# GinZhu/RDST

Measured on AMD Instinct MI355X. Metric: SR patches/sec fwd+bwd, RDST-E1 x4 64->256, higher is better.
Workload: dtype bf16; 1 GPU; RDST-E1 x4 (RDST_E1_OASIS_example_SRx4.ini), 1x64x64 LR patches -> 256x256, step = fwd + L1 + bwd + flat-bucket grad all-reduce + Adam; global_batch=32, per_gpu_batch=32, parallelism=dp1, hip_graph=True, grad_bucket_bytes=17859844

## Files before the change

### rdst_amd/csrc/mlp_mfma.hip

```cpp
#include "linear.h"
#include "mfma.h"
#include "reduce_batch.h"
#include "wattn_hd.h"
#include <stdlib.h>

#ifdef MLP_ABL
#define MLP_DBG(p) (MLP_ABL)
#else
#define MLP_DBG(p) RDST_DBGV((p).dbg)
#endif

namespace {
using namespace wahd;
using MM = Mma<bf16>;

struct MlpArgs {
  const bf16* X; int64_t ldx; const float* stats; const float* lnw; const float* lnb;
  const float* W1; const float* b1; const float* W2; const float* b2;
  const bf16* dY; int64_t lddy; bf16* dX; int64_t lddx;
  float* slab; int64_t slab_stride;
  int64_t M; int C; int hid; int64_t ntiles; int tiles_per_wg;
  unsigned long long* stamps;
  int dbg;
};

template <int NCT> struct MlpCfg {
  static constexpr int NJ = 2 * NCT, NT = 64 * NJ, CP = 32 * NCT, JP = 32 * NJ;
  static constexpr int KC = CP / 16, KJ = JP / 16, PK = CP / 8;
  static constexpr int LDW = NCT == 4 ? 336 : CP * 2 + 16, LDX = LDW, LDH = 64;
  static constexpr int OFF_W1 = 0, OFF_XH = OFF_W1 + JP * LDW, OFF_DY = OFF_XH + 32 * LDX, OFF_DH = OFF_DY + 32 * LDX,
                       OFF_B1 = OFF_DH + JP * LDH, OFF_SM = OFF_B1 + JP * 4, OFF_RED = OFF_SM + 32 * 4,
                       OFF_TAB = OFF_RED + NCT * 32 * 8, OFF_W2L = OFF_TAB + RDST_GELU_TAB_BYTES;
  static constexpr int W2L = NCT == 4 ? 3 : 0, SMEM = OFF_W2L + W2L * NJ * 1024;
};

__device__ __forceinline__ void gelu_pair(f32x2 x, f32x2& cdf, f32x2& ex) {
  const f32x2 z = x * 0.70710678118654752440f;
  f32x2 az;
  az.x = __builtin_fabsf(z.x); az.y = __builtin_fabsf(z.y);
  const f32x2 den = __builtin_elementwise_fma(az, (f32x2)(0.3275911f), (f32x2)(1.0f));
  f32x2 t;
  t.x = __builtin_amdgcn_rcpf(den.x); t.y = __builtin_amdgcn_rcpf(den.y);
  f32x2 pl = __builtin_elementwise_fma(t, (f32x2)(0.5f * 1.061405429f), (f32x2)(0.5f * -1.453152027f));
  pl = __builtin_elementwise_fma(pl, t, (f32x2)(0.5f * 1.421413741f));
  pl = __builtin_elementwise_fma(pl, t, (f32x2)(0.5f * -0.284496736f));
  pl = __builtin_elementwise_fma(pl, t, (f32x2)(0.5f * 0.254829592f));
  pl = pl * t;
  const f32x2 a2 = (z * -1.4426950408889634f) * z;
  ex.x = __builtin_amdgcn_exp2f(a2.x); ex.y = __builtin_amdgcn_exp2f(a2.y);
  const f32x2 qn = pl * ex, qp = (f32x2)(1.0f) - qn;
  cdf.x = x.x >= 0.f ? qp.x : qn.x;
  cdf.y = x.y >= 0.f ? qp.y : qn.y;
}

template <int NCT, bool SPLIT>
__global__ void __launch_bounds__(128 * NCT, 2) mlp_bwd_kernel(const MlpArgs p) {
  using CF = MlpCfg<NCT>;
  extern __shared__ __attribute__((aligned(16))) char smem[];
  constexpr int NT = CF::NT, JP = CF::JP, LDW = CF::LDW, LDX = CF::LDX, PK = CF::PK, NJ = CF::NJ;
  const int tid = threadIdx.x, lane = tid & 63, wave = __builtin_amdgcn_readfirstlane(tid >> 6), r = lane & 31, hh = lane >> 5;
  const int C = p.C, hid = p.hid;
  const int j = 32 * wave + r;
  float* b1s = reinterpret_cast<float*>(smem + CF::OFF_B1);
  float* sm = reinterpret_cast<float*>(smem + CF::OFF_SM);
  float* red = reinterpret_cast<float*>(smem + CF::OFF_RED);
  const lds_cp gtab = (lds_cp)(smem + CF::OFF_TAB);
  gelu_tab_fill(smem + CF::OFF_TAB, tid, NT);
  int nst = 0;
  auto stamp = [&]() {
    if (RDST_DBGV(p.stamps) && tid == 0 && nst < 14) p.stamps[(size_t)blockIdx.x * 16 + nst++] = __builtin_readcyclecounter();
  };
  stamp();

  Pack16 w2b[CF::KC - CF::W2L];
  const lds_cp w2l = (lds_cp)(smem + CF::OFF_W2L + (wave * 64 + lane) * 16);
  {
    float f[CF::KC][8];
#pragma unroll
    for (int t = 0; t < CF::KC; ++t)
#pragma unroll
      for (int e = 0; e < 8; ++e) {
        const int c = 16 * t + 8 * hh + e;
        f[t][e] = p.W2[(int64_t)(c < C ? c : C - 1) * hid + (j < hid ? j : hid - 1)];
      }
#pragma unroll
    for (int t = 0; t < CF::KC; ++t) {
#pragma unroll
      for (int e = 0; e < 8; ++e) f[t][e] = (16 * t + 8 * hh + e < C && j < hid) ? f[t][e] : 0.f;
      if (t < CF::KC - CF::W2L) w2b[t < CF::KC - CF::W2L ? t : 0] = MM::pack(f[t]);
      else {
        const Pack16 pk = MM::pack(f[t]);
        u32x4_t v; v.x = pk.w[0]; v.y = pk.w[1]; v.z = pk.w[2]; v.w = pk.w[3];
        *reinterpret_cast<LDS_AS u32x4_t*>(w2l + (t - (CF::KC - CF::W2L)) * NJ * 1024) = v;
      }
    }
  }
  stamp();
  lds_zero16(smem + CF::OFF_W1, CF::OFF_DH - CF::OFF_W1, tid, NT);
  const int pk = tid % PK, jr = tid / PK, c0 = 8 * pk;
  {
    float gq[8], bq[8];
#pragma unroll
    for (int e = 0; e < 8; ++e) {
      const int c = c0 + e < C ? c0 + e : C - 1;
      gq[e] = p.lnw[c];
      bq[e] = p.lnb[c];
    }
#pragma unroll
    for (int e = 0; e < 8; ++e) {
      gq[e] = c0 + e < C ? gq[e] : 0.f;
      bq[e] = c0 + e < C ? bq[e] : 0.f;
    }
    const int cl = c0 < C - 8 ? c0 : C - 8, sh = c0 - cl;
    float w[NJ][8];
#pragma unroll
    for (int ps = 0; ps < NJ; ++ps) {
      const int jj = jr + 32 * ps;
      const float* src = p.W1 + (int64_t)(jj < hid ? jj : hid - 1) * C + cl;
      const u32x4_a4 a = *reinterpret_cast<const u32x4_a4*>(src), b = *reinterpret_cast<const u32x4_a4*>(src + 4);
      w[ps][0] = __uint_as_float(a.x); w[ps][1] = __uint_as_float(a.y); w[ps][2] = __uint_as_float(a.z); w[ps][3] = __uint_as_float(a.w);
      w[ps][4] = __uint_as_float(b.x); w[ps][5] = __uint_as_float(b.y); w[ps][6] = __uint_as_float(b.z); w[ps][7] = __uint_as_float(b.w);
    }
    if (sh != 0) {
#pragma unroll
      for (int ps = 0; ps < NJ; ++ps) {
        float t4[8], t2[8];
#pragma unroll
        for (int e = 0; e < 8; ++e) t4[e] = (sh & 4) ? (e + 4 < 8 ? w[ps][e + 4 < 8 ? e + 4 : 7] : 0.f) : w[ps][e];
#pragma unroll
        for (int e = 0; e < 8; ++e) t2[e] = (sh & 2) ? (e + 2 < 8 ? t4[e + 2 < 8 ? e + 2 : 7] : 0.f) : t4[e];
#pragma unroll
        for (int e = 0; e < 8; ++e) w[ps][e] = sh >= 8 ? 0.f : t2[e];
      }
    }
    __syncthreads();
    stamp();
    float* part = reinterpret_cast<float*>(smem + CF::OFF_DH);
#pragma unroll
    for (int ps = 0; ps < NJ; ++ps) {
      const int jj = jr + 32 * ps;
      if (jj < hid) {
        float f[8], dot = 0.f;
#pragma unroll
        for (int e = 0; e < 8; ++e) {
          f[e] = w[ps][e] * gq[e];
          dot = fmaf(w[ps][e], bq[e], dot);
        }
        *reinterpret_cast<Pack16*>(smem + CF::OFF_W1 + jj * LDW + c0 * 2) = MM::pack(f);
        part[jj * PK + pk] = dot;
      }
    }
    if (tid < 32) *reinterpret_cast<uint16_t*>(smem + CF::OFF_XH + tid * LDX + C * 2) = 0x3f80;
  }
  __syncthreads();
  stamp();
  {
    const float* part = reinterpret_cast<const float*>(smem + CF::OFF_DH);
    for (int jj = tid; jj < JP; jj += NT) {
      float v = 0.f;
      if (jj < hid) {
        v = p.b1 ? p.b1[jj] : 0.f;
#pragma unroll
        for (int k = 0; k < PK; ++k) v += part[jj * PK + k];
      }
      b1s[jj] = v;
    }
  }
  __syncthreads();

  stamp();
  constexpr int NU = SPLIT ? 2 : 1;
  const bool loader = SPLIT ? wave >= NCT : true;
  const int rowbytes = C * 2;
  int lrow[NU], loff[NU];
  bool lact[NU], lal[NU], lfirst[NU];
  const char* xp[NU];
  const char* yp[NU];
  const float* sp[NU];
#pragma unroll
  for (int u = 0; u < NU; ++u) {
    const int idx = SPLIT ? (tid - 64 * NCT) + 64 * NCT * u : tid;
    lrow[u] = (idx / PK) & 31;
    const int chk = idx - (idx / PK) * PK;
    lact[u] = loader && chk * 16 < rowbytes;
    int o = chk * 16;
    if (o + 16 > rowbytes) o = rowbytes - 16;
    if (!lact[u]) o = 0;
    loff[u] = o;
    lal[u] = (o & 15) == 0;
    lfirst[u] = lact[u] && chk == 0;
  }
  u32x4_a4 rx[NU], rdy[NU];
  float2 rst[NU];
  auto seek = [&](int64_t tile) {
#pragma unroll
    for (int u = 0; u < NU; ++u) {
      int64_t row = tile * 32 + lrow[u];
      row = row < p.M ? row : p.M - 1;
      xp[u] = reinterpret_cast<const char*>(p.X + row * p.ldx) + loff[u];
      yp[u] = reinterpret_cast<const char*>(p.dY + row * p.lddy) + loff[u];
      sp[u] = p.stats + 2 * row;
    }
  };
  auto fetch = [&]() {
#pragma unroll
    for (int u = 0; u < NU; ++u) {
      rx[u] = *reinterpret_cast<const u32x4_a4*>(xp[u]);
      rdy[u] = *reinterpret_cast<const u32x4_a4*>(yp[u]);
      rst[u] = *reinterpret_cast<const float2*>(sp[u]);
    }
  };
  const int64_t xstep = 32 * p.ldx * 2, ystep = 32 * p.lddy * 2;
  auto advance = [&]() {
#pragma unroll
    for (int u = 0; u < NU; ++u) {
      xp[u] += xstep;
      yp[u] += ystep;
      sp[u] += 64;
    }
  };
  auto put16 = [&](char* dst, const Pack16& v, bool aligned) {
    if (aligned) *reinterpret_cast<Pack16*>(dst) = v;
    else {
      uint32_t* d = reinterpret_cast<uint32_t*>(dst);
      d[0] = v.w[0]; d[1] = v.w[1]; d[2] = v.w[2]; d[3] = v.w[3];
    }
  };
  auto stash = [&](int64_t tile) {
#pragma unroll
    for (int u = 0; u < NU; ++u) {
      const bool valid = tile * 32 + lrow[u] < p.M;
      if (lact[u]) {
        float f[8];
        unpack8(rx[u], f);
#pragma unroll
        for (int e = 0; e < 8; ++e) f[e] = valid ? (f[e] - rst[u].x) * rst[u].y : 0.f;
        put16(smem + CF::OFF_XH + lrow[u] * LDX + loff[u], MM::pack(f), lal[u]);
        Pack16 d;
        d.w[0] = valid ? rdy[u].x : 0u; d.w[1] = valid ? rdy[u].y : 0u; d.w[2] = valid ? rdy[u].z : 0u; d.w[3] = valid ? rdy[u].w : 0u;
        put16(smem + CF::OFF_DY + lrow[u] * LDX + loff[u], d, lal[u]);
      }
    }
#pragma unroll
    for (int u = 0; u < NU; ++u)
      if (lfirst[u]) sm[lrow[u]] = rst[u].y;
  };

  const int q = (lane & 15) >> 2, pp = lane & 3, gq1 = (lane >> 4) & 1;
  const int sg = (r & 16) + 4 * (r & 3) + ((r >> 2) & 1) + 2 * ((r >> 3) & 1);
  const lds_cp xrow = (lds_cp)(smem + CF::OFF_XH + sg * LDX + hh * 16);
  const lds_cp yrow = (lds_cp)(smem + CF::OFF_DY + sg * LDX + hh * 16);
  const lds_cp wrow = (lds_cp)(smem + CF::OFF_W1 + j * LDW + hh * 16);
  const int dhpos = 32 * wave + (r & 16) + 4 * (r & 3) + ((r >> 2) & 3);
  const uint32_t dho = (uint32_t)dhpos * CF::LDH + 8u * ((dhpos >> 1) & 7);
  const lds_cp dhb = (lds_cp)(smem + CF::OFF_DH);
  const lds_cp xtr = (lds_cp)(smem + CF::OFF_XH + (4 * q + hh) * LDX + (16 * gq1 + 4 * pp) * 2);
  const lds_cp ytr = (lds_cp)(smem + CF::OFF_DY + (4 * q + hh) * LDX + (16 * gq1 + 4 * pp) * 2);
  const lds_cp wtr = (lds_cp)(smem + CF::OFF_W1 + (4 * q + hh) * LDW + (16 * gq1 + 4 * pp) * 2 + wave * 64);
  const lds_cp dtr0 = dhb + (4 * hh + q) * CF::LDH + 8 * ((4 * gq1 + pp) ^ ((2 * hh + (q >> 1)) & 7));
  const lds_cp dtr1 = dhb + (4 * hh + 8 + q) * CF::LDH + 8 * ((4 * gq1 + pp) ^ ((2 * hh + 4 + (q >> 1)) & 7));
  static_assert(CF::LDH == 64 && CF::OFF_DH % 64 == 0, "dHp image: 64-byte rows, XOR swizzle of the 8-byte pieces");

  f32x16 G1[NCT], W2g[NCT];
#pragma unroll
  for (int ct = 0; ct < NCT; ++ct)
#pragma unroll
    for (int v = 0; v < 16; ++v) { G1[ct][v] = 0.f; W2g[ct][v] = 0.f; }

  const int64_t t0 = (int64_t)blockIdx.x * p.tiles_per_wg;
  const int64_t t1 = t0 + p.tiles_per_wg < p.ntiles ? t0 + p.tiles_per_wg : p.ntiles;
  const float invC = 1.0f / (float)C;
  const int64_t full_tiles = p.M / 32;
  if (loader && t0 < t1) {
    seek(t0);
    fetch();
  }
  for (int64_t tile = t0; tile < t1; ++tile) {
    if (loader) {
      stash(tile);
      if (tile + 1 < t1) {
        if (tile + 1 < full_tiles) advance();
        else seek(tile + 1);
      }
      fetch();
    }
    __syncthreads();
    stamp();
    Pack16 hA[2], dA[2];
    {
      f32x16 ah, ad;
      const float bj = b1s[j];
#pragma unroll
      for (int v = 0; v < 16; ++v) { ah[v] = bj; ad[v] = 0.f; }
      if (!(MLP_DBG(p) & 2))
#pragma unroll
      for (int t = 0; t < CF::KC; ++t) {
        const Pack16 xa = lds_pack(xrow + 32 * t), wb = lds_pack(wrow + 32 * t), ya = lds_pack(yrow + 32 * t);
        MM::mma(ah, xa, wb);
        if (t < CF::KC - CF::W2L) MM::mma(ad, ya, w2b[t < CF::KC - CF::W2L ? t : 0]);
        else MM::mma(ad, ya, lds_pack(w2l + (t - (CF::KC - CF::W2L)) * NJ * 1024));
      }
      const bool ones = j == hid;
#pragma unroll
      for (int s = 0; s < 2; ++s) {
        constexpr int LB = NCT == 4 ? 4 : 8;
#pragma unroll
        for (int b = 0; b < 8; b += LB) {
          float fr[LB];
          u32x2_t en[LB];
#pragma unroll
          for (int k = 0; k < LB; ++k) {
            uint32_t off;
            fr[k] = gelu_tab_index(ah[8 * s + b + k], off);
            if (MLP_DBG(p) & 1) { en[k].x = off; en[k].y = off + 1; }
            else en[k] = *reinterpret_cast<const LDS_AS u32x2_t*>(gtab + off);
          }
          __builtin_amdgcn_sched_barrier(0);
#pragma unroll
          for (int k = 0; k < LB; k += 2) {
            const int v = 8 * s + b + k;
            const float h0 = ah[v] * gelu_tab_lerp(fr[k], en[k].x), h1 = ah[v + 1] * gelu_tab_lerp(fr[k + 1], en[k + 1].x);
            const float d0 = ad[v] * gelu_tab_lerp(fr[k], en[k].y), d1 = ad[v + 1] * gelu_tab_lerp(fr[k + 1], en[k + 1].y);
            const uint32_t hp = pack_bf16x2(h0, h1);
            hA[s].w[(b + k) / 2] = ones ? 0x3f803f80u : hp;
            dA[s].w[(b + k) / 2] = pack_bf16x2(d0, d1);
          }
        }
        u32x2_t lo, hi;
        lo.x = dA[s].w[0]; lo.y = dA[s].w[1]; hi.x = dA[s].w[2]; hi.y = dA[s].w[3];
        *reinterpret_cast<LDS_AS u32x2_t*>(dhb + (dho ^ (uint32_t)(8 * (4 * s + hh)))) = lo;
        *reinterpret_cast<LDS_AS u32x2_t*>(dhb + (dho ^ (uint32_t)(8 * (4 * s + 2 + hh)))) = hi;
      }
    }
    __syncthreads();
    stamp();
    if (!(MLP_DBG(p) & 4))
#pragma unroll
    for (int ct = 0; ct < NCT; ++ct)
#pragma unroll
      for (int s = 0; s < 2; ++s) {
        const Pack16 xb = lds_tr_pack(xtr + 16 * s * LDX + ct * 64, xtr + (16 * s + 2) * LDX + ct * 64);
        const Pack16 yb = lds_tr_pack(ytr + 16 * s * LDX + ct * 64, ytr + (16 * s + 2) * LDX + ct * 64);
        MM::mma(G1[ct], dA[s], xb);
        MM::mma(W2g[ct], hA[s], yb);
      }
    f32x16 dx;
    float rstd = 0.f;
    if (wave < NCT) {
      f32x16 dx2;
#pragma unroll
      for (int v = 0; v < 16; ++v) { dx[v] = 0.f; dx2[v] = 0.f; }
      if (!(MLP_DBG(p) & 8))
#pragma unroll
      for (int kk = 0; kk < CF::KJ; kk += 2) {
        const Pack16 wa = lds_tr_pack(wtr + 16 * kk * LDW, wtr + (16 * kk + 2) * LDW);
        const Pack16 db = lds_tr_pack(dtr0 + 16 * kk * CF::LDH, dtr1 + 16 * kk * CF::LDH);
        const Pack16 wa2 = lds_tr_pack(wtr + 16 * (kk + 1) * LDW, wtr + (16 * (kk + 1) + 2) * LDW);
        const Pack16 db2 = lds_tr_pack(dtr0 + 16 * (kk + 1) * CF::LDH, dtr1 + 16 * (kk + 1) * CF::LDH);
        MM::mma(dx, wa, db);
        MM::mma(dx2, wa2, db2);
      }
#pragma unroll
      for (int v = 0; v < 16; ++v) dx[v] += dx2[v];
      rstd = sm[sg];
      float s1 = 0.f, s2 = 0.f;
#pragma unroll
      for (int g4 = 0; g4 < 4; ++g4) {
        const u32x2_t xv = *reinterpret_cast<const LDS_AS u32x2_t*>((lds_cp)(smem + CF::OFF_XH + sg * LDX) + (32 * wave + 8 * g4 + 4 * hh) * 2);
        const float xh[4] = {bf16lo(xv.x), bf16hi(xv.x), bf16lo(xv.y), bf16hi(xv.y)};
#pragma unroll
        for (int e = 0; e < 4; ++e) {
          s1 += dx[4 * g4 + e];
          s2 = fmaf(dx[4 * g4 + e], xh[e], s2);
        }
      }
      s1 = half_swap_sum(s1);
      s2 = half_swap_sum(s2);
      if (hh == 0) *reinterpret_cast<float2*>(red + (wave * 32 + r) * 2) = make_float2(s1, s2);
    }
    __syncthreads();
    stamp();
    if (wave < NCT) {
      float s1 = 0.f, s2 = 0.f;
#pragma unroll
      for (int w = 0; w < NCT; ++w) {
        const float2 v = *reinterpret_cast<const float2*>(red + (w * 32 + r) * 2);
        s1 += v.x; s2 += v.y;
      }
      s1 *= invC; s2 *= invC;
      float o[16];
#pragma unroll
      for (int g4 = 0; g4 < 4; ++g4) {
        const int cb = (32 * wave + 8 * g4 + 4 * hh) * 2;
        const u32x2_t xv = *reinterpret_cast<const LDS_AS u32x2_t*>((lds_cp)(smem + CF::OFF_XH + sg * LDX) + cb);
        const u32x2_t yv = *reinterpret_cast<const LDS_AS u32x2_t*>((lds_cp)(smem + CF::OFF_DY + sg * LDX) + cb);
        const float xh[4] = {bf16lo(xv.x), bf16hi(xv.x), bf16lo(xv.y), bf16hi(xv.y)};
        const float dy[4] = {bf16lo(yv.x), bf16hi(yv.x), bf16lo(yv.y), bf16hi(yv.y)};
#pragma unroll
        for (int e = 0; e < 4; ++e) o[4 * g4 + e] = fmaf(rstd, dx[4 * g4 + e] - s1 - xh[e] * s2, dy[e]);
      }
      const int64_t row = tile * 32 + sg;
      if (row < p.M) {
        bf16* drow = p.dX + row * p.lddx;
#pragma unroll
        for (int gp = 0; gp < 2; ++gp) {
          float c8[8];
#pragma unroll
          for (int e = 0; e < 4; ++e) {
            const auto sw = __builtin_amdgcn_permlane32_swap(__float_as_uint(o[8 * gp + e]), __float_as_uint(o[8 * gp + 4 + e]), false, false);
            c8[e] = __uint_as_float(sw[0]);
            c8[4 + e] = __uint_as_float(sw[1]);
          }
          const int cb = 32 * wave + 8 * (2 * gp + hh);
          if (cb + 8 <= C) {
            u32x4_a4 u;
            u.x = pack_bf16x2(c8[0], c8[1]); u.y = pack_bf16x2(c8[2], c8[3]);
            u.z = pack_bf16x2(c8[4], c8[5]); u.w = pack_bf16x2(c8[6], c8[7]);
            *reinterpret_cast<u32x4_a4*>(drow + cb) = u;
          } else {
#pragma unroll
            for (int e = 0; e < 8; ++e)
              if (cb + e < C) drow[cb + e] = __float2bfloat16(c8[e]);
          }
        }
      }
    }
    __syncthreads();
    stamp();
  }
  if (RDST_DBGV(p.stamps) && tid == 0) p.stamps[(size_t)blockIdx.x * 16 + 14] = __builtin_readcyclecounter();
  uint2* my = reinterpret_cast<uint2*>(p.slab) + (int64_t)blockIdx.x * p.slab_stride;
  uint2* my2 = my + (int64_t)((hid + 3) / 4) * (C + 1);
#pragma unroll
  for (int ct = 0; ct < NCT; ++ct) {
    const int c = 32 * ct + r;
#pragma unroll
    for (int g4 = 0; g4 < 4; ++g4) {
      const int j0 = 32 * wave + 8 * g4 + 4 * hh;
      if (j0 < hid && c <= C)
        my[(int64_t)(j0 >> 2) * (C + 1) + c] = make_uint2(pack_bf16x2(G1[ct][4 * g4], G1[ct][4 * g4 + 1]), pack_bf16x2(G1[ct][4 * g4 + 2], G1[ct][4 * g4 + 3]));
      if (j0 <= hid && c < C)
        my2[(int64_t)(j0 >> 2) * C + c] = make_uint2(pack_bf16x2(W2g[ct][4 * g4], W2g[ct][4 * g4 + 1]), pack_bf16x2(W2g[ct][4 * g4 + 2], W2g[ct][4 * g4 + 3]));
    }
  }
  if (RDST_DBGV(p.stamps) && tid == 0) p.stamps[(size_t)blockIdx.x * 16 + 15] = __builtin_readcyclecounter();
}

template <int NCT> struct MlpFwdCfg {
  static constexpr int NJ = 2 * NCT, NT = 64 * NJ, CP = 32 * NCT, JP = 32 * NJ;
  static constexpr int KC = CP / 16, KJ = JP / 16, PK = CP / 8;
  static constexpr int LDW = CP * 2 + 16, LDX = CP * 2 + 16, LD2 = JP * 2 + 16;
  static constexpr int off_w2(int hid) { return hid * LDW; }
  static constexpr int off_x(int hid, int C) { return off_w2(hid) + C * LD2; }
  static constexpr int off_h(int hid, int C) { return off_x(hid, C) + 32 * LDX; }
  static constexpr int off_pst(int hid, int C) { return off_h(hid, C) + 32 * LD2; }
  static constexpr int off_s(int hid, int C) { return off_pst(hid, C) + 32 * 16 * 8; }
  static constexpr int smem(int hid, int C) { return off_s(hid, C) + 2 * JP * 4 + CP * 4; }
};

struct MlpFwdArgs {
  const bf16* X; int64_t ldx; const float* lnw; const float* lnb;
  const float* W1; const float* b1; const float* W2; const float* b2;
  bf16* Y; int64_t ldy; float* stats;
  int64_t M; int C; int hid; int64_t ntiles; int tiles_per_wg;
  unsigned long long* stamps;
};

template <int NCT>
__global__ void __launch_bounds__(128 * NCT, 2) mlp_fwd_kernel(const MlpFwdArgs p) {
  using CF = MlpFwdCfg<NCT>;
  extern __shared__ __attribute__((aligned(16))) char smem[];
  constexpr int NT = CF::NT, JP = CF::JP, CP = CF::CP, LDW = CF::LDW, LDX = CF::LDX, LD2 = CF::LD2, PK = CF::PK, NJ = CF::NJ;
  const int tid = threadIdx.x, lane = tid & 63, wave = __builtin_amdgcn_readfirstlane(tid >> 6), r = lane & 31, hh = lane >> 5;
  const int C = p.C, hid = p.hid;
  const int OFF_W2 = CF::off_w2(hid), OFF_X = CF::off_x(hid, C), OFF_H = CF::off_h(hid, C), OFF_PST = CF::off_pst(hid, C),
            OFF_S = CF::off_s(hid, C);
  float* Ss = reinterpret_cast<float*>(smem + OFF_S);
  float* b1s = Ss + JP;
  float* b2s = b1s + JP;
  float2* pst = reinterpret_cast<float2*>(smem + OFF_PST);
  int nst = 0;
  auto stamp = [&]() {
    if (RDST_DBGV(p.stamps) && tid == 0 && nst < 16) p.stamps[(size_t)blockIdx.x * 16 + nst++] = __builtin_readcyclecounter();
  };
  stamp();

  lds_zero16(smem, OFF_H, tid, NT);
  const int pk = tid % PK, jr = tid / PK, c0 = 8 * pk;
  {
    float gq[8], bq[8];
#pragma unroll
    for (int e = 0; e < 8; ++e) {
      const int c = c0 + e < C ? c0 + e : C - 1;
      gq[e] = p.lnw[c];
      bq[e] = p.lnb[c];
    }
// ... 204 lines not shown
        const int kc = 2 * k + hh;
        const bool last = kc == nchunk - 1;
        const float d = q2[k].x * (last ? inv_nlast : 0.125f) - mean;
        m2 += kc < nchunk ? fmaf((last ? (float)nlast : 8.0f) * d, d, q2[k].y) : 0.f;
      }
      m2 = half_swap_sum(m2);
#pragma unroll
      for (int v = 0; v < 16; ++v) ah[v] += ah2[v];
      const float rstd = 1.0f / sqrtf(m2 * invC + 1e-5f);
      const int64_t row = tile * 32 + r;
      if (wave == 0 && hh == 0 && row < p.M) *reinterpret_cast<float2*>(p.stats + 2 * row) = make_float2(mean, rstd);
      const float nm = -mean * rstd;
#pragma unroll
      for (int g4 = 0; g4 < 4; ++g4) {
        const float sq[4] = {Sr[4 * g4], Sr[4 * g4 + 1], Sr[4 * g4 + 2], Sr[4 * g4 + 3]};
        const float bq[4] = {B1r[4 * g4], B1r[4 * g4 + 1], B1r[4 * g4 + 2], B1r[4 * g4 + 3]};
        float hv[4];
#pragma unroll
        for (int e2 = 0; e2 < 2; ++e2) {
          f32x2 x, cdf, ex;
          x.x = fmaf(ah[4 * g4 + 2 * e2], rstd, fmaf(nm, sq[2 * e2], bq[2 * e2]));
          x.y = fmaf(ah[4 * g4 + 2 * e2 + 1], rstd, fmaf(nm, sq[2 * e2 + 1], bq[2 * e2 + 1]));
          gelu_pair(x, cdf, ex);
          hv[2 * e2] = x.x * cdf.x;
          hv[2 * e2 + 1] = x.y * cdf.y;
        }
        u32x2_t w2;
        w2.x = pack_bf16x2(hv[0], hv[1]); w2.y = pack_bf16x2(hv[2], hv[3]);
        *reinterpret_cast<LDS_AS u32x2_t*>(hwr + 16 * g4) = w2;
      }
    }
    __syncthreads();
    stamp();
    if (wave < NCT) {
      f32x16 y0, y1;
#pragma unroll
      for (int v = 0; v < 16; ++v) { y0[v] = B2r[v]; y1[v] = 0.f; }
#pragma unroll
      for (int kk = 0; kk < CF::KJ; kk += 2) {
        const Pack16 wa = lds_pack(w2row + 32 * kk), hb = lds_pack(hrd + 32 * kk);
        const Pack16 wa2 = lds_pack(w2row + 32 * (kk + 1)), hb2 = lds_pack(hrd + 32 * (kk + 1));
        MM::mma(y0, wa, hb);
        MM::mma(y1, wa2, hb2);
      }
      float o[16];
#pragma unroll
      for (int g4 = 0; g4 < 4; ++g4) {
        const u32x2_t xv = *reinterpret_cast<const LDS_AS u32x2_t*>((lds_cp)(smem + OFF_X + r * LDX) + (j0 + 8 * g4 + 4 * hh) * 2);
        const float xr[4] = {bf16lo(xv.x), bf16hi(xv.x), bf16lo(xv.y), bf16hi(xv.y)};
#pragma unroll
        for (int e = 0; e < 4; ++e) o[4 * g4 + e] = y0[4 * g4 + e] + y1[4 * g4 + e] + xr[e];
      }
      const int64_t row = tile * 32 + r;
      if (row < p.M) {
        bf16* yrow = p.Y + row * p.ldy;
#pragma unroll
        for (int gp = 0; gp < 2; ++gp) {
          float c8[8];
#pragma unroll
          for (int e = 0; e < 4; ++e) {
            const auto sw = __builtin_amdgcn_permlane32_swap(__float_as_uint(o[8 * gp + e]), __float_as_uint(o[8 * gp + 4 + e]), false, false);
            c8[e] = __uint_as_float(sw[0]);
            c8[4 + e] = __uint_as_float(sw[1]);
          }
          const int cb = j0 + 8 * (2 * gp + hh);
          if (cb + 8 <= C) {
            u32x4_a4 u;
            u.x = pack_bf16x2(c8[0], c8[1]); u.y = pack_bf16x2(c8[2], c8[3]);
            u.z = pack_bf16x2(c8[4], c8[5]); u.w = pack_bf16x2(c8[6], c8[7]);
            *reinterpret_cast<u32x4_a4*>(yrow + cb) = u;
          } else {
#pragma unroll
            for (int e = 0; e < 8; ++e)
              if (cb + e < C) yrow[cb + e] = __float2bfloat16(c8[e]);
          }
        }
      }
    }
    __syncthreads();
    stamp();
  }
}

int mlp_nct(int C, int hid) {
  const int nct = (C + 1 + 31) / 32;
  if (nct < 2 || nct > 4) return 0;
  if (hid + 1 > 64 * nct || hid < 32) return 0;
  if ((C & 1) || C * 2 < 16) return 0;
  const int fs = nct == 2 ? MlpFwdCfg<2>::smem(hid, C) : nct == 3 ? MlpFwdCfg<3>::smem(hid, C) : MlpFwdCfg<4>::smem(hid, C);
  if (fs > 160 * 1024) return 0;
  return nct;
}

bool mlp_fused(int C, int hid) {
  static int off = -1;
  if (off < 0) {
    const char* e = rdst_dbg_getenv("RDST_MLP_V1");
    off = (e && e[0] == '1') ? 1 : 0;
  }
  return !off && mlp_nct(C, hid) != 0;
}

}

extern "C" int rdst_mlp_fused_supported(int C, int hid, int dtype) {
  if (rdst_dtype(dtype, "rdst_mlp_fused_supported")) return 0;
  return dtype == RDST_BF16 && mlp_fused(C, hid);
}

namespace {
struct MlpBwdWs {
  WsSlab slab;
  float* G;
  size_t bytes;
};
MlpBwdWs mlp_bwd_layout(void* base, int C, int hid) {
  WsCarver c(base);
  MlpBwdWs w{};
  w.slab = ws_take_slab(c, 2 * kCUs, (int64_t)hid * (C + 1) + (int64_t)(hid + 1) * C);
  w.G = c.take<float>((size_t)hid * (C + 1) + kWsSlackFloats);
  w.bytes = c.bytes();
  return w;
}
}

extern "C" size_t rdst_mlp_bwd_workspace(int64_t M, int C, int hid) {
  (void)M;
  if (C <= 0 || hid <= 0) return 0;
  return mlp_bwd_layout(nullptr, C, hid).bytes;
}

extern "C" int rdst_mlp_bwd(const void* X, int64_t ld_x, const float* ln_w, const float* ln_b, const float* stats,
                            const float* W1, const float* b1, const float* W2, const void* dY, int64_t ld_dy, void* dX,
                            int64_t ld_dx, float* dW1, float* db1, float* dW2, float* db2, float* dln_w, float* dln_b,
                            void* workspace, size_t workspace_bytes, int64_t M, int C, int hid, int dtype, void* stream) {
  if (int rc = rdst_dtype(dtype, "rdst_mlp_bwd")) return rc;
  if (!X || !ln_w || !ln_b || !stats || !W1 || !W2 || !dY || !dX || !dW1 || !db1 || !dW2 || !db2 || !dln_w || !dln_b || !workspace)
    return rdst_fail(RDST_EINVAL, "rdst_mlp_bwd: null pointer");
  if (M < 0 || C <= 0 || hid <= 0 || ld_x < C || ld_dy < C || ld_dx < C) return rdst_fail(RDST_EINVAL, "rdst_mlp_bwd: bad dimensions");
  if (dtype != RDST_BF16 || !mlp_fused(C, hid)) return RDST_ENOTSUP;
  if (((uintptr_t)X & 3) || ((uintptr_t)dY & 3) || ((uintptr_t)dX & 3) || (ld_x & 1) || (ld_dy & 1) || (ld_dx & 1)) return RDST_ENOTSUP;
  if (workspace_bytes < rdst_mlp_bwd_workspace(M, C, hid)) return rdst_fail(RDST_EINVAL, "rdst_mlp_bwd: workspace too small");
  if (M == 0) return 0;
  hipStream_t st = (hipStream_t)stream;
  const int nct = mlp_nct(C, hid);
  MlpArgs p{};
  p.X = (const bf16*)X; p.ldx = ld_x; p.stats = stats; p.lnw = ln_w; p.lnb = ln_b; p.W1 = W1; p.b1 = b1; p.W2 = W2;
  p.dY = (const bf16*)dY; p.lddy = ld_dy; p.dX = (bf16*)dX; p.lddx = ld_dx;
  p.M = M; p.C = C; p.hid = hid;
  p.ntiles = (M + 31) / 32;
  int64_t cap = nct == 2 ? 2 * kCUs : kCUs;
  { const char* e = rdst_dbg_getenv("RDST_MLP_GRID"); if (e && atoi(e) > 0) cap = atoi(e); }
  const MlpBwdWs w = mlp_bwd_layout(workspace, C, hid);
  p.slab = w.slab.p;
  p.slab_stride = (int64_t)((hid + 3) / 4) * (C + 1) + (int64_t)((hid + 4) / 4) * C;
  const int64_t grid = rdst_tile_grid(p.ntiles, w.slab.cap(cap, 2 * p.slab_stride), &p.tiles_per_wg);
  if (int rc = rdst_slab_fits(w.slab, grid, 2 * p.slab_stride, "mlp_bwd")) return rc;
  float* const G = w.G;
  int rc = 0;
#define RDST_MLPB(NC)                                                                                                \
  {                                                                                                                  \
    auto kern = split ? mlp_bwd_kernel<NC, true> : mlp_bwd_kernel<NC, false>;                                                                                \
    constexpr int smem = MlpCfg<NC>::SMEM;                                                                           \
    rc = rdst_launch(kern, dim3((unsigned)grid), dim3(128 * NC), smem, st, "mlp_bwd", p);                             \
  }
  static int split = -1;
  if (split < 0) { const char* e = rdst_dbg_getenv("RDST_MLP_SPLIT"); split = (e && e[0] == '1') ? 1 : 0; }
  { const char* e = rdst_dbg_getenv("RDST_MLP_DBG"); p.dbg = e ? atoi(e) : 0; }
  p.stamps = rdst_stamps_begin("RDST_MLP_STAMPS", grid, 16, st);
  if (nct == 2) RDST_MLPB(2) else if (nct == 3) RDST_MLPB(3) else RDST_MLPB(4)
#undef RDST_MLPB
  rdst_stamps_end(p.stamps, grid, 16, RDST_STAMPS_TICKS, st, "mlp_bwd C=%d hid=%d", C, hid);
  if (rc) return rc;
  const int tot = (int)p.slab_stride;
  {
    (void)tot;
    rbatch::SumJob s1{};
    s1.slab = p.slab; s1.nwg = (int)grid; s1.stride = p.slab_stride; s1.g4 = 1; s1.a2 = hid; s1.b2 = C + 1;
    s1.tot = ((hid + 3) / 4) * (C + 1); s1.map = rbatch::MAP_COPY; s1.out = G;
    if (int rc = rbatch::sum(s1, st)) return rc;
    rbatch::SumJob s2{};
    s2.slab = p.slab + 2 * (int64_t)((hid + 3) / 4) * (C + 1); s2.nwg = (int)grid; s2.stride = p.slab_stride; s2.g4 = 1;
    s2.a2 = hid + 1; s2.b2 = C; s2.tot = ((hid + 4) / 4) * C; s2.map = rbatch::MAP_T; s2.out = dW2; s2.out2 = db2; s2.a = hid;
    if (int rc = rbatch::sum(s2, st)) return rc;
  }
  return wgrad_ln_finish_launch(G, W1, ln_w, ln_b, hid, C, 1.0f, dW1, db1, dln_w, dln_b, st);
}

extern "C" size_t rdst_mlp_fwd_workspace(int C, int hid) {
  if (C <= 0 || hid <= 0) return 16;
  return mlp3_pack_bytes(C, hid);
}
extern "C" int rdst_mlp_fwd_packable(int C, int hid, int dtype) {
  if (rdst_dtype(dtype, "rdst_mlp_fwd_packable")) return 0;
  return dtype == RDST_BF16 && mlp3_fwd_shape(C, hid);
}

extern "C" int rdst_mlp_fwd(const void* X, int64_t ld_x, const float* ln_w, const float* ln_b, const float* W1, const float* b1,
                            const float* W2, const float* b2, void* Y, int64_t ld_y, float* stats, void* workspace,
                            size_t workspace_bytes, int64_t M, int C, int hid, int dtype, void* stream) {
  if (int rc = rdst_dtype(dtype, "rdst_mlp_fwd")) return rc;
  if (!X || !ln_w || !ln_b || !W1 || !W2 || !Y || !stats) return rdst_fail(RDST_EINVAL, "rdst_mlp_fwd: null pointer");
  if (M < 0 || C <= 0 || hid <= 0 || ld_x < C || ld_y < C) return rdst_fail(RDST_EINVAL, "rdst_mlp_fwd: bad dimensions");
  if (dtype != RDST_BF16 || !mlp_fused(C, hid)) return RDST_ENOTSUP;
  if (((uintptr_t)X & 3) || ((uintptr_t)Y & 3) || (ld_x & 1) || (ld_y & 1) || hid < 8) return RDST_ENOTSUP;
  if (M == 0) return 0;
  hipStream_t st = (hipStream_t)stream;
  if (workspace && workspace_bytes >= rdst_mlp_fwd_workspace(C, hid)) {
    const int rc = mlp3_fwd_bf16((const bf16*)X, ld_x, ln_w, ln_b, W1, b1, W2, b2, (bf16*)Y, ld_y, stats, M, C, hid, workspace,
                                 workspace_bytes == RDST_PREPACKED, st);
    if (rc != RDST_ENOTSUP) return rc;
  }
  const int nct = mlp_nct(C, hid);
  MlpFwdArgs p{};
  p.X = (const bf16*)X; p.ldx = ld_x; p.lnw = ln_w; p.lnb = ln_b; p.W1 = W1; p.b1 = b1; p.W2 = W2; p.b2 = b2;
  p.Y = (bf16*)Y; p.ldy = ld_y; p.stats = stats; p.M = M; p.C = C; p.hid = hid;
  p.ntiles = (M + 31) / 32;
  int64_t cap = nct == 2 ? 2 * kCUs : kCUs;
  { const char* e = rdst_dbg_getenv("RDST_MLP_GRID"); if (e && atoi(e) > 0) cap = atoi(e); }
  const int64_t grid = rdst_tile_grid(p.ntiles, cap, &p.tiles_per_wg);
  int rc = 0;
#define RDST_MLPF(NC)                                                                                                \
  {                                                                                                                  \
    auto kern = mlp_fwd_kernel<NC>;                                                                                  \
    const int smem = MlpFwdCfg<NC>::smem(hid, C);                                                                    \
    if (smem > 160 * 1024) return RDST_ENOTSUP;                                                                      \
    rc = rdst_launch(kern, dim3((unsigned)grid), dim3(128 * NC), smem, st, "mlp_fwd", p);                             \
  }
  p.stamps = rdst_stamps_begin("RDST_MLPF_STAMPS", grid, 16, st);
  if (nct == 2) RDST_MLPF(2) else if (nct == 3) RDST_MLPF(3) else RDST_MLPF(4)
#undef RDST_MLPF
  rdst_stamps_end(p.stamps, grid, 16, RDST_STAMPS_TICKS, st, "mlp_fwd C=%d hid=%d", C, hid);
  return rc;
}
```

Before: 1937 patches/s.

## Process two 32-row tiles per iteration in fused MLP backward kernel

Adds a PAIR variant of the fused MLP backward kernel. Each loop iteration stages two 32-row tiles in LDS, so the otherwise idle upper half of the waves can compute dX for the second tile while the lower waves handle the first. Loads for the next pair are prefetched, and for NCT=3 the second prefetch is deferred until after the barrier. This is meant to cut idle waves and the number of barriers per tile, at the cost of more LDS and registers, which may lower occupancy. It is enabled by default for NCT 2 and 3 and can be turned off with an environment variable.

```diff
diff --git a/rdst_amd/csrc/mlp_mfma.hip b/rdst_amd/csrc/mlp_mfma.hip
--- a/rdst_amd/csrc/mlp_mfma.hip
+++ b/rdst_amd/csrc/mlp_mfma.hip
@@ -24,14 +24,14 @@
   int dbg;
 };
 
-template <int NCT> struct MlpCfg {
+template <int NCT, int NTL = 1> struct MlpCfg {
   static constexpr int NJ = 2 * NCT, NT = 64 * NJ, CP = 32 * NCT, JP = 32 * NJ;
   static constexpr int KC = CP / 16, KJ = JP / 16, PK = CP / 8;
   static constexpr int LDW = NCT == 4 ? 336 : CP * 2 + 16, LDX = LDW, LDH = 64;
-  static constexpr int OFF_W1 = 0, OFF_XH = OFF_W1 + JP * LDW, OFF_DY = OFF_XH + 32 * LDX, OFF_DH = OFF_DY + 32 * LDX,
-                       OFF_B1 = OFF_DH + JP * LDH, OFF_SM = OFF_B1 + JP * 4, OFF_RED = OFF_SM + 32 * 4,
-                       OFF_TAB = OFF_RED + NCT * 32 * 8, OFF_W2L = OFF_TAB + RDST_GELU_TAB_BYTES;
-  static constexpr int W2L = NCT == 4 ? 3 : 0, SMEM = OFF_W2L + W2L * NJ * 1024;
+  static constexpr int OFF_W1 = 0, OFF_XH = OFF_W1 + JP * LDW, OFF_DY = OFF_XH + NTL * 32 * LDX,
+                       OFF_DH = OFF_DY + NTL * 32 * LDX, OFF_B1 = OFF_DH + NTL * JP * LDH, OFF_SM = OFF_B1 + JP * 4,
+                       OFF_RED = OFF_SM + NTL * 32 * 4, OFF_TAB = OFF_RED + NTL * NCT * 32 * 8, OFF_W2L = OFF_TAB + RDST_GELU_TAB_BYTES;
+  static constexpr int W2L = NCT == 4 ? 3 : (NCT == 3 && NTL == 2) ? 2 : 0, SMEM = OFF_W2L + W2L * NJ * 1024;
 };
 
 __device__ __forceinline__ void gelu_pair(f32x2 x, f32x2& cdf, f32x2& ex) {
@@ -53,9 +53,11 @@
   cdf.y = x.y >= 0.f ? qp.y : qn.y;
 }
 
-template <int NCT, bool SPLIT>
+template <int NCT, bool SPLIT, bool PAIR>
 __global__ void __launch_bounds__(128 * NCT, 2) mlp_bwd_kernel(const MlpArgs p) {
-  using CF = MlpCfg<NCT>;
+  constexpr int NTL = PAIR ? 2 : 1;
+  constexpr bool B_LATE = NCT == 3;
+  using CF = MlpCfg<NCT, NTL>;
   extern __shared__ __attribute__((aligned(16))) char smem[];
   constexpr int NT = CF::NT, JP = CF::JP, LDW = CF::LDW, LDX = CF::LDX, PK = CF::PK, NJ = CF::NJ;
   const int tid = threadIdx.x, lane = tid & 63, wave = __builtin_amdgcn_readfirstlane(tid >> 6), r = lane & 31, hh = lane >> 5;
@@ -150,7 +152,7 @@
         part[jj * PK + pk] = dot;
       }
     }
-    if (tid < 32) *reinterpret_cast<uint16_t*>(smem + CF::OFF_XH + tid * LDX + C * 2) = 0x3f80;
+    if (tid < 32 * NTL) *reinterpret_cast<uint16_t*>(smem + CF::OFF_XH + tid * LDX + C * 2) = 0x3f80;
   }
   __syncthreads();
   stamp();
@@ -174,9 +176,9 @@
   const int rowbytes = C * 2;
   int lrow[NU], loff[NU];
   bool lact[NU], lal[NU], lfirst[NU];
-  const char* xp[NU];
-  const char* yp[NU];
-  const float* sp[NU];
+  const char* xp[NTL][NU];
+  const char* yp[NTL][NU];
+  const float* sp[NTL][NU];
 #pragma unroll
   for (int u = 0; u < NU; ++u) {
     const int idx = SPLIT ? (tid - 64 * NCT) + 64 * NCT * u : tid;
@@ -190,33 +192,33 @@
     lal[u] = (o & 15) == 0;
     lfirst[u] = lact[u] && chk == 0;
   }
-  u32x4_a4 rx[NU], rdy[NU];
-  float2 rst[NU];
-  auto seek = [&](int64_t tile) {
+  u32x4_a4 rx[NTL][NU], rdy[NTL][NU];
+  float2 rst[NTL][NU];
+  auto seek = [&](int b, int64_t tile) {
 #pragma unroll
     for (int u = 0; u < NU; ++u) {
       int64_t row = tile * 32 + lrow[u];
       row = row < p.M ? row : p.M - 1;
-      xp[u] = reinterpret_cast<const char*>(p.X + row * p.ldx) + loff[u];
-      yp[u] = reinterpret_cast<const char*>(p.dY + row * p.lddy) + loff[u];
-      sp[u] = p.stats + 2 * row;
+      xp[b][u] = reinterpret_cast<const char*>(p.X + row * p.ldx) + loff[u];
+      yp[b][u] = reinterpret_cast<const char*>(p.dY + row * p.lddy) + loff[u];
+      sp[b][u] = p.stats + 2 * row;
     }
   };
-  auto fetch = [&]() {
+  auto fetch = [&](int b) {
 #pragma unroll
     for (int u = 0; u < NU; ++u) {
-      rx[u] = *reinterpret_cast<const u32x4_a4*>(xp[u]);
-      rdy[u] = *reinterpret_cast<const u32x4_a4*>(yp[u]);
-      rst[u] = *reinterpret_cast<const float2*>(sp[u]);
+      rx[b][u] = *reinterpret_cast<const u32x4_a4*>(xp[b][u]);
+      rdy[b][u] = *reinterpret_cast<const u32x4_a4*>(yp[b][u]);
+      rst[b][u] = *reinterpret_cast<const float2*>(sp[b][u]);
     }
   };
   const int64_t xstep = 32 * p.ldx * 2, ystep = 32 * p.lddy * 2;
-  auto advance = [&]() {
+  auto advance = [&](int b) {
 #pragma unroll
     for (int u = 0; u < NU; ++u) {
-      xp[u] += xstep;
-      yp[u] += ystep;
-      sp[u] += 64;
+      xp[b][u] += xstep;
+      yp[b][u] += ystep;
+      sp[b][u] += 64;
     }
   };
   auto put16 = [&](char* dst, const Pack16& v, bool aligned) {
@@ -226,24 +228,24 @@
       d[0] = v.w[0]; d[1] = v.w[1]; d[2] = v.w[2]; d[3] = v.w[3];
     }
   };
-  auto stash = [&](int64_t tile) {
+  auto stash = [&](int b, int64_t tile) {
 #pragma unroll
     for (int u = 0; u < NU; ++u) {
       const bool valid = tile * 32 + lrow[u] < p.M;
       if (lact[u]) {
         float f[8];
-        unpack8(rx[u], f);
-#pragma unroll
-        for (int e = 0; e < 8; ++e) f[e] = valid ? (f[e] - rst[u].x) * rst[u].y : 0.f;
-        put16(smem + CF::OFF_XH + lrow[u] * LDX + loff[u], MM::pack(f), lal[u]);
+        unpack8(rx[b][u], f);
+#pragma unroll
+        for (int e = 0; e < 8; ++e) f[e] = valid ? (f[e] - rst[b][u].x) * rst[b][u].y : 0.f;
+        put16(smem + CF::OFF_XH + (32 * b + lrow[u]) * LDX + loff[u], MM::pack(f), lal[u]);
         Pack16 d;
-        d.w[0] = valid ? rdy[u].x : 0u; d.w[1] = valid ? rdy[u].y : 0u; d.w[2] = valid ? rdy[u].z : 0u; d.w[3] = valid ? rdy[u].w : 0u;
-        put16(smem + CF::OFF_DY + lrow[u] * LDX + loff[u], d, lal[u]);
+        d.w[0] = valid ? rdy[b][u].x : 0u; d.w[1] = valid ? rdy[b][u].y : 0u; d.w[2] = valid ? rdy[b][u].z : 0u; d.w[3] = valid ? rdy[b][u].w : 0u;
+        put16(smem + CF::OFF_DY + (32 * b + lrow[u]) * LDX + loff[u], d, lal[u]);
       }
     }
 #pragma unroll
     for (int u = 0; u < NU; ++u)
-      if (lfirst[u]) sm[lrow[u]] = rst[u].y;
+      if (lfirst[u]) sm[32 * b + lrow[u]] = rst[b][u].y;
   };
 
   const int q = (lane & 15) >> 2, pp = lane & 3, gq1 = (lane >> 4) & 1;
@@ -256,7 +258,9 @@
   const lds_cp dhb = (lds_cp)(smem + CF::OFF_DH);
   const lds_cp xtr = (lds_cp)(smem + CF::OFF_XH + (4 * q + hh) * LDX + (16 * gq1 + 4 * pp) * 2);
   const lds_cp ytr = (lds_cp)(smem + CF::OFF_DY + (4 * q + hh) * LDX + (16 * gq1 + 4 * pp) * 2);
-  const lds_cp wtr = (lds_cp)(smem + CF::OFF_W1 + (4 * q + hh) * LDW + (16 * gq1 + 4 * pp) * 2 + wave * 64);
+  const int b3 = PAIR && wave >= NCT ? 1 : 0, w3 = wave - NCT * b3;
+  const int o3x = b3 * 32 * LDX, o3h = b3 * JP * CF::LDH;
+  const lds_cp wtr = (lds_cp)(smem + CF::OFF_W1 + (4 * q + hh) * LDW + (16 * gq1 + 4 * pp) * 2 + w3 * 64);
   const lds_cp dtr0 = dhb + (4 * hh + q) * CF::LDH + 8 * ((4 * gq1 + pp) ^ ((2 * hh + (q >> 1)) & 7));
   const lds_cp dtr1 = dhb + (4 * hh + 8 + q) * CF::LDH + 8 * ((4 * gq1 + pp) ^ ((2 * hh + 4 + (q >> 1)) & 7));
   static_assert(CF::LDH == 64 && CF::OFF_DH % 64 == 0, "dHp image: 64-byte rows, XOR swizzle of the 8-byte pieces");
@@ -272,81 +276,106 @@
   const float invC = 1.0f / (float)C;
   const int64_t full_tiles = p.M / 32;
   if (loader && t0 < t1) {
-    seek(t0);
-    fetch();
-  }
-  for (int64_t tile = t0; tile < t1; ++tile) {
+    seek(0, t0);
+    fetch(0);
+    if constexpr (PAIR) {
+      seek(1, t0 + 1);
+      fetch(1);
+    }
+  }
+  for (int64_t tile = t0; tile < t1; tile += NTL) {
+    const bool two = PAIR && tile + 1 < t1;
     if (loader) {
-      stash(tile);
-      if (tile + 1 < t1) {
-        if (tile + 1 < full_tiles) advance();
-        else seek(tile + 1);
-      }
-      fetch();
+      stash(0, tile);
+      if constexpr (PAIR) {
+        if (two) stash(1, tile + 1);
+        if constexpr (!B_LATE) {
+          seek(1, tile + 3);
+          fetch(1);
+        }
+        seek(0, tile + 2);
+      } else if (tile + 1 < t1) {
+        if (tile + 1 < full_tiles) advance(0);
+        else seek(0, tile + 1);
+      }
+      fetch(0);
     }
     __syncthreads();
     stamp();
-    Pack16 hA[2], dA[2];
-    {
-      f32x16 ah, ad;
-      const float bj = b1s[j];
-#pragma unroll
-      for (int v = 0; v < 16; ++v) { ah[v] = bj; ad[v] = 0.f; }
-      if (!(MLP_DBG(p) & 2))
-#pragma unroll
-      for (int t = 0; t < CF::KC; ++t) {
-        const Pack16 xa = lds_pack(xrow + 32 * t), wb = lds_pack(wrow + 32 * t), ya = lds_pack(yrow + 32 * t);
-        MM::mma(ah, xa, wb);
-        if (t < CF::KC - CF::W2L) MM::mma(ad, ya, w2b[t < CF::KC - CF::W2L ? t : 0]);
-        else MM::mma(ad, ya, lds_pack(w2l + (t - (CF::KC - CF::W2L)) * NJ * 1024));
-      }
-      const bool ones = j == hid;
-#pragma unroll
-      for (int s = 0; s < 2; ++s) {
-        constexpr int LB = NCT == 4 ? 4 : 8;
-#pragma unroll
-        for (int b = 0; b < 8; b += LB) {
-          float fr[LB];
-          u32x2_t en[LB];
-#pragma unroll
-          for (int k = 0; k < LB; ++k) {
-            uint32_t off;
-            fr[k] = gelu_tab_index(ah[8 * s + b + k], off);
-            if (MLP_DBG(p) & 1) { en[k].x = off; en[k].y = off + 1; }
-            else en[k] = *reinterpret_cast<const LDS_AS u32x2_t*>(gtab + off);
+    Pack16 hA[NTL][2], dA[NTL][2];
+    auto phase2 = [&](int tb) {
+      if (!(MLP_DBG(p) & 4))
+#pragma unroll
+      for (int ct = 0; ct < NCT; ++ct)
+#pragma unroll
+        for (int s = 0; s < 2; ++s) {
+          const Pack16 xb = lds_tr_pack(xtr + (32 * tb + 16 * s) * LDX + ct * 64, xtr + (32 * tb + 16 * s + 2) * LDX + ct * 64);
+          const Pack16 yb = lds_tr_pack(ytr + (32 * tb + 16 * s) * LDX + ct * 64, ytr + (32 * tb + 16 * s + 2) * LDX + ct * 64);
+          MM::mma(G1[ct], dA[tb][s], xb);
+          MM::mma(W2g[ct], hA[tb][s], yb);
+        }
+    };
+#pragma unroll
+    for (int tb = 0; tb < NTL; ++tb)
+      if (tb == 0 || two) {
+        f32x16 ah, ad;
+        const float bj = b1s[j];
+#pragma unroll
+        for (int v = 0; v < 16; ++v) { ah[v] = bj; ad[v] = 0.f; }
+        if (!(MLP_DBG(p) & 2))
+#pragma unroll
+        for (int t = 0; t < CF::KC; ++t) {
+          const Pack16 xa = lds_pack(xrow + tb * 32 * LDX + 32 * t), wb = lds_pack(wrow + 32 * t), ya = lds_pack(yrow + tb * 32 * LDX + 32 * t);
+          MM::mma(ah, xa, wb);
+          if (t < CF::KC - CF::W2L) MM::mma(ad, ya, w2b[t < CF::KC - CF::W2L ? t : 0]);
+          else MM::mma(ad, ya, lds_pack(w2l + (t - (CF::KC - CF::W2L)) * NJ * 1024));
+        }
+        const bool ones = j == hid;
+#pragma unroll
+        for (int s = 0; s < 2; ++s) {
+          constexpr int LB = NCT == 4 ? 4 : 8;
+#pragma unroll
+          for (int b = 0; b < 8; b += LB) {
+            float fr[LB];
+            u32x2_t en[LB];
+#pragma unroll
+            for (int k = 0; k < LB; ++k) {
+              uint32_t off;
+              fr[k] = gelu_tab_index(ah[8 * s + b + k], off);
+              if (MLP_DBG(p) & 1) { en[k].x = off; en[k].y = off + 1; }
+              else en[k] = *reinterpret_cast<const LDS_AS u32x2_t*>(gtab + off);
+            }
+            __builtin_amdgcn_sched_barrier(0);
+#pragma unroll
+            for (int k = 0; k < LB; k += 2) {
+              const int v = 8 * s + b + k;
+              const float h0 = ah[v] * gelu_tab_lerp(fr[k], en[k].x), h1 = ah[v + 1] * gelu_tab_lerp(fr[k + 1], en[k + 1].x);
+              const float d0 = ad[v] * gelu_tab_lerp(fr[k], en[k].y), d1 = ad[v + 1] * gelu_tab_lerp(fr[k + 1], en[k + 1].y);
+              const uint32_t hp = pack_bf16x2(h0, h1);
+              hA[tb][s].w[(b + k) / 2] = ones ? 0x3f803f80u : hp;
+              dA[tb][s].w[(b + k) / 2] = pack_bf16x2(d0, d1);
+            }
           }
-          __builtin_amdgcn_sched_barrier(0);
-#pragma unroll
-          for (int k = 0; k < LB; k += 2) {
-            const int v = 8 * s + b + k;
-            const float h0 = ah[v] * gelu_tab_lerp(fr[k], en[k].x), h1 = ah[v + 1] * gelu_tab_lerp(fr[k + 1], en[k + 1].x);
-            const float d0 = ad[v] * gelu_tab_lerp(fr[k], en[k].y), d1 = ad[v + 1] * gelu_tab_lerp(fr[k + 1], en[k + 1].y);
-            const uint32_t hp = pack_bf16x2(h0, h1);
-            hA[s].w[(b + k) / 2] = ones ? 0x3f803f80u : hp;
-            dA[s].w[(b + k) / 2] = pack_bf16x2(d0, d1);
-          }
-        }
-        u32x2_t lo, hi;
-        lo.x = dA[s].w[0]; lo.y = dA[s].w[1]; hi.x = dA[s].w[2]; hi.y = dA[s].w[3];
-        *reinterpret_cast<LDS_AS u32x2_t*>(dhb + (dho ^ (uint32_t)(8 * (4 * s + hh)))) = lo;
-        *reinterpret_cast<LDS_AS u32x2_t*>(dhb + (dho ^ (uint32_t)(8 * (4 * s + 2 + hh)))) = hi;
-      }
-    }
+          u32x2_t lo, hi;
+          lo.x = dA[tb][s].w[0]; lo.y = dA[tb][s].w[1]; hi.x = dA[tb][s].w[2]; hi.y = dA[tb][s].w[3];
+          *reinterpret_cast<LDS_AS u32x2_t*>(dhb + tb * JP * CF::LDH + (dho ^ (uint32_t)(8 * (4 * s + hh)))) = lo;
+          *reinterpret_cast<LDS_AS u32x2_t*>(dhb + tb * JP * CF::LDH + (dho ^ (uint32_t)(8 * (4 * s + 2 + hh)))) = hi;
+        }
+        if constexpr (PAIR) if (tb == 0) phase2(0);
+      }
     __syncthreads();
     stamp();
-    if (!(MLP_DBG(p) & 4))
-#pragma unroll
-    for (int ct = 0; ct < NCT; ++ct)
-#pragma unroll
-      for (int s = 0; s < 2; ++s) {
-        const Pack16 xb = lds_tr_pack(xtr + 16 * s * LDX + ct * 64, xtr + (16 * s + 2) * LDX + ct * 64);
-        const Pack16 yb = lds_tr_pack(ytr + 16 * s * LDX + ct * 64, ytr + (16 * s + 2) * LDX + ct * 64);
-        MM::mma(G1[ct], dA[s], xb);
-        MM::mma(W2g[ct], hA[s], yb);
-      }
+    if constexpr (PAIR && B_LATE)
+      if (loader) {
+        seek(1, tile + 3);
+        fetch(1);
+      }
+    if constexpr (PAIR) { if (two) phase2(1); }
+    else phase2(0);
+    const bool act3 = PAIR ? (b3 == 0 || two) : wave < NCT;
     f32x16 dx;
     float rstd = 0.f;
-    if (wave < NCT) {
+    if (act3) {
       f32x16 dx2;
 #pragma unroll
       for (int v = 0; v < 16; ++v) { dx[v] = 0.f; dx2[v] = 0.f; }
@@ -354,19 +383,19 @@
 #pragma unroll
       for (int kk = 0; kk < CF::KJ; kk += 2) {
         const Pack16 wa = lds_tr_pack(wtr + 16 * kk * LDW, wtr + (16 * kk + 2) * LDW);
-        const Pack16 db = lds_tr_pack(dtr0 + 16 * kk * CF::LDH, dtr1 + 16 * kk * CF::LDH);
+        const Pack16 db = lds_tr_pack(dtr0 + o3h + 16 * kk * CF::LDH, dtr1 + o3h + 16 * kk * CF::LDH);
         const Pack16 wa2 = lds_tr_pack(wtr + 16 * (kk + 1) * LDW, wtr + (16 * (kk + 1) + 2) * LDW);
-        const Pack16 db2 = lds_tr_pack(dtr0 + 16 * (kk + 1) * CF::LDH, dtr1 + 16 * (kk + 1) * CF::LDH);
+        const Pack16 db2 = lds_tr_pack(dtr0 + o3h + 16 * (kk + 1) * CF::LDH, dtr1 + o3h + 16 * (kk + 1) * CF::LDH);
         MM::mma(dx, wa, db);
         MM::mma(dx2, wa2, db2);
       }
 #pragma unroll
       for (int v = 0; v < 16; ++v) dx[v] += dx2[v];
-      rstd = sm[sg];
+      rstd = sm[32 * b3 + sg];
       float s1 = 0.f, s2 = 0.f;
 #pragma unroll
       for (int g4 = 0; g4 < 4; ++g4) {
-        const u32x2_t xv = *reinterpret_cast<const LDS_AS u32x2_t*>((lds_cp)(smem + CF::OFF_XH + sg * LDX) + (32 * wave + 8 * g4 + 4 * hh) * 2);
+        const u32x2_t xv = *reinterpret_cast<const LDS_AS u32x2_t*>((lds_cp)(smem + CF::OFF_XH + o3x + sg * LDX) + (32 * w3 + 8 * g4 + 4 * hh) * 2);
         const float xh[4] = {bf16lo(xv.x), bf16hi(xv.x), bf16lo(xv.y), bf16hi(xv.y)};
 #pragma unroll
         for (int e = 0; e < 4; ++e) {
@@ -380,26 +409,26 @@
     }
     __syncthreads();
     stamp();
-    if (wave < NCT) {
+    if (act3) {
       float s1 = 0.f, s2 = 0.f;
 #pragma unroll
       for (int w = 0; w < NCT; ++w) {
-        const float2 v = *reinterpret_cast<const float2*>(red + (w * 32 + r) * 2);
+        const float2 v = *reinterpret_cast<const float2*>(red + ((NCT * b3 + w) * 32 + r) * 2);
         s1 += v.x; s2 += v.y;
       }
       s1 *= invC; s2 *= invC;
       float o[16];
 #pragma unroll
       for (int g4 = 0; g4 < 4; ++g4) {
-        const int cb = (32 * wave + 8 * g4 + 4 * hh) * 2;
-        const u32x2_t xv = *reinterpret_cast<const LDS_AS u32x2_t*>((lds_cp)(smem + CF::OFF_XH + sg * LDX) + cb);
-        const u32x2_t yv = *reinterpret_cast<const LDS_AS u32x2_t*>((lds_cp)(smem + CF::OFF_DY + sg * LDX) + cb);
+        const int cb = (32 * w3 + 8 * g4 + 4 * hh) * 2;
+        const u32x2_t xv = *reinterpret_cast<const LDS_AS u32x2_t*>((lds_cp)(smem + CF::OFF_XH + o3x + sg * LDX) + cb);
+        const u32x2_t yv = *reinterpret_cast<const LDS_AS u32x2_t*>((lds_cp)(smem + CF::OFF_DY + o3x + sg * LDX) + cb);
         const float xh[4] = {bf16lo(xv.x), bf16hi(xv.x), bf16lo(xv.y), bf16hi(xv.y)};
         const float dy[4] = {bf16lo(yv.x), bf16hi(yv.x), bf16lo(yv.y), bf16hi(yv.y)};
 #pragma unroll
         for (int e = 0; e < 4; ++e) o[4 * g4 + e] = fmaf(rstd, dx[4 * g4 + e] - s1 - xh[e] * s2, dy[e]);
       }
-      const int64_t row = tile * 32 + sg;
+      const int64_t row = (tile + b3) * 32 + sg;
       if (row < p.M) {
         bf16* drow = p.dX + row * p.lddx;
 #pragma unroll
@@ -411,7 +440,7 @@
             c8[e] = __uint_as_float(sw[0]);
             c8[4 + e] = __uint_as_float(sw[1]);
           }
-          const int cb = 32 * wave + 8 * (2 * gp + hh);
+          const int cb = 32 * w3 + 8 * (2 * gp + hh);
           if (cb + 8 <= C) {
             u32x4_a4 u;
             u.x = pack_bf16x2(c8[0], c8[1]); u.y = pack_bf16x2(c8[2], c8[3]);
@@ -782,6 +811,9 @@
   }
 }
 
+static_assert(2 * MlpCfg<2, 2>::SMEM <= 160 * 1024 && MlpCfg<3, 2>::SMEM <= 160 * 1024 && MlpCfg<4, 2>::SMEM > 160 * 1024,
+              "mlp_bwd pair loop: LDS budget");
+
 int mlp_nct(int C, int hid) {
   const int nct = (C + 1 + 31) / 32;
   if (nct < 2 || nct > 4) return 0;
@@ -858,17 +890,21 @@
   if (int rc = rdst_slab_fits(w.slab, grid, 2 * p.slab_stride, "mlp_bwd")) return rc;
   float* const G = w.G;
   int rc = 0;
-#define RDST_MLPB(NC)                                                                                                \
+#define RDST_MLPB(NC, PR)                                                                                              \
   {                                                                                                                  \
-    auto kern = split ? mlp_bwd_kernel<NC, true> : mlp_bwd_kernel<NC, false>;                                                                                \
-    constexpr int smem = MlpCfg<NC>::SMEM;                                                                           \
+    auto kern = split ? mlp_bwd_kernel<NC, true, false> : mlp_bwd_kernel<NC, false, PR>;                             \
+    constexpr int smem = MlpCfg<NC, PR ? 2 : 1>::SMEM;                                                               \
     rc = rdst_launch(kern, dim3((unsigned)grid), dim3(128 * NC), smem, st, "mlp_bwd", p);                             \
   }
   static int split = -1;
   if (split < 0) { const char* e = rdst_dbg_getenv("RDST_MLP_SPLIT"); split = (e && e[0] == '1') ? 1 : 0; }
   { const char* e = rdst_dbg_getenv("RDST_MLP_DBG"); p.dbg = e ? atoi(e) : 0; }
   p.stamps = rdst_stamps_begin("RDST_MLP_STAMPS", grid, 16, st);
-  if (nct == 2) RDST_MLPB(2) else if (nct == 3) RDST_MLPB(3) else RDST_MLPB(4)
+  static const bool pair_on = [] { const char* e = getenv("RDST_MLP_BWD_PAIR"); return !(e && e[0] == '0'); }();
+  const bool pair = pair_on && !split;
+  if (nct == 2) { if (pair) RDST_MLPB(2, true) else RDST_MLPB(2, false) }
+  else if (nct == 3) { if (pair) RDST_MLPB(3, true) else RDST_MLPB(3, false) }
+  else RDST_MLPB(4, false)
 #undef RDST_MLPB
   rdst_stamps_end(p.stamps, grid, 16, RDST_STAMPS_TICKS, st, "mlp_bwd C=%d hid=%d", C, hid);
   if (rc) return rc;
```

After: 1951 patches/s, median of 6. Within noise of the previous version (+0.7%).
